# yixuan/ADMM

Hardware: AMD Instinct MI355X
Metric: ADMM iterations/sec, Lasso tall n=100000 p=10000 (100-lambda warm-started path) (higher is better)
Workload: dtype f32; 1 GPU; admm_lasso tall path (BASELINE configs[1]); n=100000, p=10000, nlambda=100, standardize=True, intercept=True, parallelism=single GPU, step=one cold-started warm-chained lambda path

## Files before the change

admm_amd/_lib.py:

```python
import ctypes
import os

import numpy as np

_HERE = os.path.dirname(os.path.abspath(__file__))
LIB_PATH = os.environ.get("ADMM_HIP_LIB") or os.path.join(_HERE, "lib", "libadmm_hip.so")

ADMM_MEM_HOST = 0
ADMM_MEM_DEVICE = 1


class AdmmOpts(ctypes.Structure):
    _fields_ = [("maxit", ctypes.c_int), ("eps_abs", ctypes.c_double),
                ("eps_rel", ctypes.c_double), ("rho", ctypes.c_double)]


class AdmmHipOptions(ctypes.Structure):
    _fields_ = [(k, ctypes.c_int) for k in (
        "struct_size", "gram_backend", "gram_split", "factor_backend", "inverse_precision", "tall_xupdate", "tall_refine",
        "consensus_two_pass", "consensus_unfused", "bp_two_pass", "lad_no_hat", "wide_no_persist", "wide_unfused", "wide_gram_sprad",
        "sharing_bp_direct", "cv_downdate", "peer_exchange", "batch_iters", "profile_stride", "pool_mb", "screen", "lad_two_pass",
        "par_devices")] + [("reserved", ctypes.c_int * 9)]


# ... 30 lines not shown
           "admm_hip_device_synchronize", "admm_hip_lasso_plan_create", "admm_hip_lasso_plan_run",
           "admm_hip_lasso_plan_destroy", "admm_hip_comm_unique_id", "admm_hip_comm_init", "admm_hip_comm_finalize", "admm_hip_comm_info",
           "admm_hip_parlasso_dist", "admm_hip_lasso_plan_create_dist",
           "admm_hip_lasso_plan_trace_enable", "admm_hip_lasso_plan_trace_read",
           "admm_hip_lasso_plan_state_enable", "admm_hip_lasso_plan_state_read", "admm_hip_lasso_plan_system_read",
           "admm_hip_host_lanczos", "admm_hip_test_symv",
           "admm_hip_comm_peer_prepare", "admm_hip_comm_init_peer", "admm_hip_comm_init_shm", "admm_hip_comm_test_allreduce", "admm_hip_comm_test_reduce_scatter",
           "admm_hip_lasso_dist", "admm_hip_test_gram", "admm_hip_test_spd_inverse", "admm_hip_test_cv_fold_system",
           "admm_hip_lasso_dist_cols", "admm_hip_test_gemv_t", "admm_hip_lad_traced", "admm_hip_bp_traced",
           "admm_hip_lasso_plan_create_dist_cols", "admm_hip_lasso_cv", "admm_hip_lasso_multi",
           "admm_hip_parbp", "admm_hip_parbp_traced", "admm_hip_parbp_dist", "admm_hip_dantzig", "admm_hip_dantzig_traced",
           "admm_hip_lad_state", "admm_hip_bp_state", "admm_hip_lasso_plan_data_read", "admm_hip_trim_memory", "admm_hip_test_gather",
           "admm_hip_options_default", "admm_hip_options_set", "admm_hip_option_set", "admm_hip_options_reset", "admm_hip_option_get",
           "admm_hip_last_parallel_layout", "admm_hip_parallel_assign", "admm_hip_grplasso", "admm_hip_grplasso_plan_create",
           "admm_hip_quantreg", "admm_hip_quantreg_state",
           "admm_hip_mtlasso", "admm_hip_mtlasso_plan_create", "admm_hip_test_symv_multi"]

GROUP_MAX = 1024
MT_MAX = 16
MT_RHS_BUILT = (2, 4, 8, 12)

TRACE_FIELDS = 12
TRACE_COLD, TRACE_CONVERGED, TRACE_ACCELERATE, TRACE_RESTART = -1, 0, 1, 2
TRACE_CONTINUE = 1


def load():
    global _lib
    if _lib is not None:
        return _lib
    path = os.environ.get("ADMM_HIP_LIB") or LIB_PATH
# ... 127 lines not shown
    lib.admm_hip_lasso_plan_trace_read.argtypes = [ctypes.c_void_p, _c_double_p, ctypes.c_longlong, ctypes.POINTER(ctypes.c_longlong)]
    lib.admm_hip_lasso_plan_trace_read.restype = ctypes.c_int
    lib.admm_hip_lasso_plan_state_enable.argtypes = [ctypes.c_void_p, ctypes.c_longlong]
    lib.admm_hip_lasso_plan_state_enable.restype = ctypes.c_int
    lib.admm_hip_lasso_plan_state_read.argtypes = [ctypes.c_void_p, ctypes.POINTER(ctypes.c_float), ctypes.c_longlong,
                                                   ctypes.POINTER(ctypes.c_longlong), ctypes.POINTER(ctypes.c_longlong)]
    lib.admm_hip_lasso_plan_state_read.restype = ctypes.c_int
    lib.admm_hip_lasso_plan_data_read.argtypes = [ctypes.c_void_p, ctypes.POINTER(ctypes.c_float), ctypes.c_longlong, ctypes.POINTER(ctypes.c_float)]
    lib.admm_hip_lasso_plan_data_read.restype = ctypes.c_int
    lib.admm_hip_lasso_plan_system_read.argtypes = [ctypes.c_void_p, ctypes.POINTER(ctypes.c_float), ctypes.c_longlong]
    lib.admm_hip_lasso_plan_system_read.restype = ctypes.c_int
    lib.admm_hip_test_symv.argtypes = [_c_float_p, ctypes.c_int, _c_float_p, _c_float_p, _c_float_p, _c_float_p]
    lib.admm_hip_test_symv.restype = ctypes.c_int
    lib.admm_hip_test_symv_multi.argtypes = [_c_float_p, ctypes.c_int, _c_float_p, ctypes.c_int, ctypes.c_int, _c_float_p]
    lib.admm_hip_test_symv_multi.restype = ctypes.c_int
    lib.admm_hip_test_gram.argtypes = [ctypes.c_void_p, ctypes.c_int, ctypes.c_int, ctypes.c_int, ctypes.c_int, ctypes.c_void_p]
    lib.admm_hip_test_gram.restype = ctypes.c_int
    lib.admm_hip_test_gemv_t.argtypes = [ctypes.c_void_p, ctypes.c_int, ctypes.c_int, ctypes.c_int, ctypes.c_void_p, ctypes.c_void_p]
    lib.admm_hip_test_gemv_t.restype = ctypes.c_int
    lib.admm_hip_test_spd_inverse.argtypes = [ctypes.c_void_p, ctypes.c_int, ctypes.c_int, ctypes.c_void_p]
    lib.admm_hip_test_spd_inverse.restype = ctypes.c_int
    lib.admm_hip_test_cv_fold_system.argtypes = [ctypes.c_void_p, ctypes.c_void_p, ctypes.c_int, ctypes.c_int, ctypes.c_void_p, ctypes.c_int, ctypes.c_int,
                                                 ctypes.c_int, ctypes.c_int, ctypes.c_void_p, ctypes.c_void_p, ctypes.c_void_p, ctypes.c_void_p, ctypes.c_void_p]
    lib.admm_hip_test_cv_fold_system.restype = ctypes.c_int
    lib.admm_hip_host_lanczos.argtypes = [_c_float_p, ctypes.c_int, _c_float_p, _c_int_p]
    lib.admm_hip_host_lanczos.restype = ctypes.c_int
    lib.admm_hip_test_gather.argtypes = [ctypes.c_void_p, ctypes.c_int, ctypes.c_int, ctypes.c_int, ctypes.c_void_p, _c_double_p]
    lib.admm_hip_test_gather.restype = ctypes.c_int
    lib.admm_hip_last_parallel_layout.argtypes = [_c_int_p, _c_int_p, ctypes.c_int]
    lib.admm_hip_last_parallel_layout.restype = ctypes.c_int
# ... 87 lines not shown
```

admm_amd/csrc/api.hip:

```cpp
#include "calls.h"
#include "comm.h"
#include "inproc.h"
#include "test_hooks.h"

using namespace admm;

template <typename F>
static int guarded(F&& f) {
    try {
        check_option_overlay();
        f();
        return ADMM_OK;
    } catch (const Error& e) {
        set_last_error(e.what());
        return e.code;
    } catch (const std::bad_alloc&) {
        set_last_error("host allocation failed");
        return ADMM_ERR_INTERNAL;
    } catch (const std::exception& e) {
        set_last_error(e.what());
        return ADMM_ERR_INTERNAL;
    }
}

// ... 468 lines not shown

int admm_hip_test_symv(const float* A, int p, const float* v0, const float* v1, float* y0, float* y1) {
    return guarded([&] {
        ADMM_REQUIRE(A && v0 && v1 && y0 && y1 && p > 0, "bad arguments");
        test_symv(A, p, v0, v1, y0, y1);
    });
}

int admm_hip_test_symv_multi(const float* A, int p, const float* V, int nr, int rhs_per_pass, float* Yout) {
    return guarded([&] {
        ADMM_REQUIRE(A && V && Yout && p > 0 && nr >= 1 && nr <= 64, "bad arguments");
        test_symv_multi(A, p, V, nr, rhs_per_pass, Yout);
    });
}

int admm_hip_test_gram(const void* A, int rows, int cols, int atA, int is_double, void* G) {
    return guarded([&] {
        ADMM_REQUIRE(A && G && rows > 0 && cols > 0, "bad arguments");
        if (is_double) test_gram<double>(static_cast<const double*>(A), rows, cols, atA != 0, static_cast<double*>(G));
        else test_gram<float>(static_cast<const float*>(A), rows, cols, atA != 0, static_cast<float*>(G));
    });
}

int admm_hip_test_gemv_t(const void* A, int rows, int cols, int is_double, const void* v, void* y) {
    return guarded([&] {
        ADMM_REQUIRE(A && v && y && rows > 0 && cols > 0, "bad arguments");
        if (is_double) test_gemv_t<double>(static_cast<const double*>(A), rows, cols, static_cast<const double*>(v), static_cast<double*>(y));
        else test_gemv_t<float>(static_cast<const float*>(A), rows, cols, static_cast<const float*>(v), static_cast<float*>(y));
    });
}
// ... 24 lines not shown
```

admm_amd/csrc/lasso_tall.hip:

```cpp
#include "prep.h"
#include "gemv_kernels.h"
#include "symv_kernels.h"
#include "solvers.h"
#include "comm.h"
#include "loop_driver.h"
#include "plan_host.h"
#include "peer_device.h"
#include "probe.h"

namespace admm {

struct TallCtl {
    double rho, lam, eps_primal, eps_dual, adj_a, adj_c, tau;
    double a_next, tau_next;
    int mode;
    int restart;
    int iter;
    int lam_idx;
    int done;
    int first;
    int total;
    int fin_idx;
    int fin_niter;
    int pad;
// ... 11 lines not shown
    float* x; float* z0; float* z1; float* y0; float* y1; float* adj_z; float* adj_y; float* u; float* w;
    TallCtl* ctl;
    double* P;
    float* beta;
    int* niter;
    int* done_host;
#ifdef ADMM_HIP_PROBE
    long long* probe;
#endif
    double* trace;
    long long trace_cap;
    const float* refine_ab;
    long long refine_ld;
    float* state;
    long long state_cap;
};

constexpr int kTailThreads = 256;
constexpr int kTailLanes = kSySumLanes;
constexpr int kTailElems = kTailThreads / kTailLanes;

__device__ __forceinline__ double tall_load_partial(const double* p, bool in_launch) {
    if (!in_launch) return *p;
    return __longlong_as_double((long long)__hip_atomic_load(reinterpret_cast<const unsigned long long*>(p), __ATOMIC_RELAXED, __HIP_MEMORY_SCOPE_AGENT));
}
__device__ __forceinline__ void tall_store_wt(float* p, float v) {
    __hip_atomic_store(reinterpret_cast<unsigned int*>(p), __float_as_uint(v), __ATOMIC_RELAXED, __HIP_MEMORY_SCOPE_AGENT);
}
__device__ __forceinline__ void tall_store_wt(double* p, double v) {
    __hip_atomic_store(reinterpret_cast<unsigned long long*>(p), (unsigned long long)__double_as_longlong(v), __ATOMIC_RELAXED, __HIP_MEMORY_SCOPE_AGENT);
}
// ... 46 lines not shown
            out.mode = 1;
            out.iter = in.iter + 1;
            if (in.iter + 1 >= q.maxit) {
                out.fin_idx = in.lam_idx; out.fin_niter = q.maxit + 1;
            }
        }
        if (out.fin_idx >= 0) {
            out.lam_idx = in.lam_idx + 1;
            out.iter = 0;
            if (out.lam_idx >= q.nlam) out.done = 1;
            else out.lam = q.lambdas[out.lam_idx];
            q.niter[out.fin_idx] = out.fin_niter;
        }
    } else {
        out.mode = 1; out.tau = 0.0; out.restart = 0;
    }
    out.eps_primal = fmax(sqrt(x2), sqrt(z2)) * q.eps_rel + q.sqrt_p * q.eps_abs;
    out.eps_dual = sqrt(y2) * q.eps_rel + q.sqrt_p * q.eps_abs;
    out.a_next = 0.5 + 0.5 * sqrt(1.0 + 4.0 * out.adj_a * out.adj_a);
    out.tau_next = (out.adj_a - 1.0) / out.a_next;
    out.total = in.total + 1;
    *outp = out;
    if (out.done) *q.done_host = 1;
    WIDE_PROBE(3);
    WIDE_PROBE_FLUSH(2, in.total);
    if (q.trace != nullptr && in.total < q.trace_cap) {
        double* t = q.trace + (size_t)in.total * ADMM_TRACE_FIELDS;
        t[0] = in.lam_idx; t[1] = in.iter; t[2] = in.eps_primal; t[3] = in.eps_dual; t[4] = tr_rp; t[5] = tr_rd;
        t[6] = tr_c; t[7] = in.adj_c; t[8] = tr_code; t[9] = in.rho; t[10] = in.rho; t[11] = in.lam;
    }
// ... 425 lines not shown

__global__ void tall_init_kernel(TallParams q, double rho, double lam0) {
    const int i = blockIdx.x * blockDim.x + threadIdx.x;
    if (i < q.p) {
        q.x[i] = 0.f; q.z0[i] = 0.f; q.z1[i] = 0.f; q.y0[i] = 0.f; q.y1[i] = 0.f;
        q.adj_z[i] = 0.f; q.adj_y[i] = 0.f; q.u[i] = q.XY[i]; q.w[i] = 0.f;
    }
    if (i < 2 * q.nwg * 8) q.P[i] = 0.0;
    if (i == 0) {
        TallCtl c;
        c.rho = rho; c.lam = lam0; c.eps_primal = 0.0; c.eps_dual = 0.0;
        c.adj_a = 1.0; c.adj_c = 9999.0; c.tau = 0.0;
        c.a_next = 0.5 + 0.5 * sqrt(5.0); c.tau_next = 0.0;
        c.mode = 1; c.restart = 0; c.iter = 0; c.lam_idx = 0; c.done = 0; c.first = 1; c.total = 0; c.fin_idx = -1; c.fin_niter = 0; c.pad = 0;
        q.ctl[0] = c; q.ctl[1] = c;
    }
}

struct TallPlan final : LassoPlan {
    DeviceData<float> d;
    LassoProblem pb;
    hipStream_t st;
    admm_stats setup_stats{};
    int p = 0, nlam = 0, nwg = 0;
    long long ldp = 0;
    double rho = 0;
    std::vector<double> lam_user, lam_int;
    GemvTPlan pl;
    SymvPlan sy;
    bool use_sym = false;
    bool shard = false;
    bool peer_fused = false;
    bool peer_one = false;
    int exchange_code = 0;
    CommInfo ci;
    DevBuf<float> ab;
    double dist_flops = 0;
    long long ldv = 0;
    DevBuf<float> XY, M, a_part, b_part, x, z0, z1, y0, y1, adj_z, adj_y, u, w, beta;
    DevBuf<int> niter;
    DevBuf<double> P, dlam;
    DevBuf<TallCtl> ctl;
    TallParams q{};
    bool refine = false;
    DevBuf<float> Mg, rab, ruw;
    DevBuf<double> dD0, dD1, xD0, xD1;
    bool grouped = false;
    DevBuf<int2> gtiles;
    DevBuf<GroupCoord> gcoord;
    GroupTailParams gq{};
    int mt = 0;
    int mt_rhs = 2;
    DevBuf<float> uw, mdot, maxp;
    DevBuf<double> roww;
    MtTailParams mq{};
    PinnedFlag hflag;
#ifdef ADMM_HIP_PROBE
// ... 186 lines not shown
        u.zero(st); w.zero(st);
        ADMM_HIP_CHECK(hipMemcpyAsync(dlam.get(), lam_int.data(), nlam * sizeof(double), hipMemcpyHostToDevice, st));

        q.p = p; q.nwg = nwg; q.nseg = pl.nseg; q.maxit = pb.opts.maxit; q.nlam = nlam; q.enet = pb.enet ? 1 : 0;
        q.part_stride = ldp;
        q.eps_abs = pb.opts.eps_abs; q.eps_rel = pb.opts.eps_rel; q.alpha = (double)(float)pb.alpha; q.sqrt_p = std::sqrt((double)p * (double)npl);
        q.lambdas = dlam.get(); q.XY = XY.get(); q.a_part = a_part.get(); q.b_part = b_part.get();
        if (shard) { q.a_part = ab.get(); q.b_part = ab.get() + ldp; q.nseg = 1; }
        q.dot0 = sy.dot0.get(); q.dot1 = sy.dot1.get(); q.axp0 = sy.axp0.get(); q.axp1 = sy.axp1.get();
        q.ldo = sy.ldo; q.nrb = sy.nrb; q.p32 = sy.p32; q.sched = sy.sched;
        q.refine_ab = refine ? rab.get() : nullptr; q.refine_ld = ldv;
        q.x = x.get(); q.z0 = z0.get(); q.z1 = z1.get(); q.y0 = y0.get(); q.y1 = y1.get();
        q.adj_z = adj_z.get(); q.adj_y = adj_y.get(); q.u = u.get(); q.w = w.get();
        q.ctl = ctl.get(); q.P = P.get(); q.beta = beta.get(); q.niter = niter.get();
        q.done_host = hflag.p;
#ifdef ADMM_HIP_PROBE
        probe.alloc((size_t)4096 * 4 * 8); probe.zero(st);
        q.probe = probe.get();
        sy.probe = probe.get();
#endif

        if (mt) {
            static const int kAutoRhs[kMtMax] = {2, 4, 8, 8, 12, 12, 8, 8, 4, 4, 12, 12, 4, 4, 8, 8};
            mt_rhs = kAutoRhs[mt - 1];
            if (const OptValue* v = opt(Opt::MT_RHS)) { if (v->i > 0) mt_rhs = kSyNR[v->i - 1]; }
            uw.alloc((size_t)2 * mt * ldv); uw.zero(st);
            const size_t ds = (size_t)sy.nrb * sy.ldo, as = (size_t)sy.nax_rows * sy.ldo;
            mdot.alloc((size_t)2 * mt * ds); maxp.alloc((size_t)2 * mt * as);
            mdot.zero(st); maxp.zero(st);
            x.zero(st); z0.zero(st); z1.zero(st); y0.zero(st); y1.zero(st); adj_z.zero(st); adj_y.zero(st);
// ... 63 lines not shown

    void read_system(float* out, long long ld) override {
        if (!refine) throw Error(ADMM_ERR_INVALID_ARG, "the system matrix is only kept with ADMM_HIP_REFINE=1");
        ADMM_REQUIRE(out != nullptr && ld >= p, "bad output for the system matrix");
        ADMM_HIP_CHECK(hipMemcpy2D(out, (size_t)ld * sizeof(float), Mg.get(), (size_t)ldp * sizeof(float), (size_t)p * sizeof(float), (size_t)p, hipMemcpyDeviceToHost));
    }

    void run(LassoResult& res) override {
        admm_stats S = setup_stats;
        S.xupdate_variant = shard ? 2 : (use_sym ? 1 : 0);
        S.exchange_variant = exchange_code;
        S.refine = refine ? 1 : 0;
        S.factor_flops = dist_flops;
        res.lambda = lam_user;
        beta.zero(st); niter.zero(st);
        const int init_n = std::max(p, 2 * nwg * 8);
        for (int k = 0; k < std::max(mt, 1); ++k) {
            TallParams qk = q;
            if (mt) {
                const size_t o = (size_t)k * ldv;
                qk.x += o; qk.z0 += o; qk.z1 += o; qk.y0 += o; qk.y1 += o; qk.adj_z += o; qk.adj_y += o;
                qk.XY += (size_t)k * ldp; qk.u = uw.get() + (size_t)(2 * k) * ldv; qk.w = uw.get() + (size_t)(2 * k + 1) * ldv;
            }
            hipLaunchKernelGGL(tall_init_kernel, dim3((init_n + 255) / 256), dim3(256), 0, st, qk, rho, lam_int[0]);
        }
        if (q.state != nullptr && mt)
            ADMM_HIP_CHECK(hipMemcpy2DAsync(q.state, (size_t)p * sizeof(float), XY.get(), (size_t)ldp * sizeof(float), (size_t)p * sizeof(float),
                                            (size_t)mt, hipMemcpyDeviceToDevice, st));
        else if (q.state != nullptr)
            ADMM_HIP_CHECK(hipMemcpyAsync(q.state, XY.get(), (size_t)p * sizeof(float), hipMemcpyDeviceToDevice, st));
// ... 7 lines not shown
        size_t nev = 0;
        const auto done_at = [&](long long g) -> const int* { return &ctl.get()[(int)(g & 1)].done; };
        const LoopTimes lt = run_until_done(st, done_at, batch, (long long)nlam * ((long long)pb.opts.maxit + 2) + 4, [&](long long g) {
            const int par = (int)(g & 1);
            const bool sample = stride > 0 && (g % stride) == stride / 2 && nev < 8192;
            hipEvent_t e0 = nullptr, e1 = nullptr;
            if (sample) {
                while (ev_pool.size() < nev + 2) {
                    hipEvent_t e; ADMM_HIP_CHECK(hipEventCreate(&e));
                    ev_pool.push_back(e);
                }
                e0 = ev_pool[nev]; e1 = ev_pool[nev + 1];
                nev += 2;
            }
            const TallDecideExtra dec{q, par};
            if (mt) {
                const int nvec = 2 * mt;
                for (int r0 = 0; r0 < nvec; r0 += mt_rhs) {
                    SymvNArgs a;
                    a.A = M.get(); a.lda = ldp; a.p = p;
                    a.v = uw.get() + (size_t)r0 * ldv; a.vstride = ldv;
                    a.dot = mdot.get() + (size_t)r0 * mq.dot_stride; a.dot_stride = mq.dot_stride;
                    a.axp = maxp.get() + (size_t)r0 * mq.axp_stride; a.axp_stride = mq.axp_stride;
                    a.nvec = std::min(mt_rhs, nvec - r0); a.ldo = sy.ldo; a.tiles = sy.tiles.get(); a.skip = &ctl.get()[par].done;
                    hipEvent_t es = r0 == 0 ? e0 : nullptr, ee = r0 + mt_rhs >= nvec ? e1 : nullptr;
                    if (r0 == 0) symvn_launch(sy, mt_rhs, a, st, dec, es, ee);
                    else symvn_launch(sy, mt_rhs, a, st, SymvNoExtra(), es, ee);
                }
                hipLaunchKernelGGL(tall_mt_tail_kernel, dim3(nwg), dim3(kTailThreads), 0, st, q, par, mq);
            } else if (grouped) {
                if (use_sym) {
                    sy.launch(M.get(), ldp, u.get(), w.get(), &ctl.get()[par].done, st, dec, e0, e1);
                    hipLaunchKernelGGL(tall_group_tail_kernel<TAIL_SYMV>, dim3(nwg), dim3(kTailThreads), 0, st, q, par, gq);
                } else {
                    launch_gemv_t<float, 2, 4, TallDecideExtra>(pl, M.get(), ldp, p, p, u.get(), w.get(), a_part.get(), b_part.get(), ldp,
                                                                &ctl.get()[par].done, st, dec, e0, e1);
                    hipLaunchKernelGGL(tall_group_tail_kernel<TAIL_GEMV>, dim3(nwg), dim3(kTailThreads), 0, st, q, par, gq);
                }
            } else if (shard && peer_fused) {
                sy.launch(M.get(), ldp, u.get(), w.get(), &ctl.get()[par].done, st, dec, e0, e1);
                const PeerExchange ex = comm_peer_begin((size_t)2 * ldp * sizeof(float));
                if (peer_one) {
                    hipLaunchKernelGGL(tall_tail_kernel<TAIL_PEER1>, dim3(nwg), dim3(kTailThreads), 0, st, q, par, ex);
                } else {
                    hipLaunchKernelGGL(tall_shard_push_kernel, dim3(nwg), dim3(kTailThreads), 0, st, q, ex, ldp, &ctl.get()[par].done);
                    hipLaunchKernelGGL(tall_tail_kernel<TAIL_PEER>, dim3(nwg), dim3(kTailThreads), 0, st, q, par, ex);
                }
// ... 3 lines not shown
                allreduce_sum_f32(ab.get(), (size_t)2 * ldp, st);
                hipLaunchKernelGGL(tall_tail_kernel<TAIL_GEMV>, dim3(nwg), dim3(kTailThreads), 0, st, q, par, PeerExchange{});
            } else if (use_sym && refine) {
                const int* skip = &ctl.get()[par].done;
                sy.launch(M.get(), ldp, u.get(), w.get(), skip, st, dec, e0, e1);
                hipLaunchKernelGGL(tall_shard_reduce_kernel, dim3(nwg), dim3(kTailThreads), 0, st, q, rab.get(), ldv, skip);
                SymvArgsD ad;
                ad.A = Mg.get(); ad.lda = ldp; ad.p = p; ad.v0 = rab.get(); ad.v1 = rab.get() + ldv;
                ad.dot0 = dD0.get(); ad.dot1 = dD1.get(); ad.axp0 = xD0.get(); ad.axp1 = xD1.get(); ad.ldo = sy.ldo; ad.tiles = sy.tiles.get(); ad.skip = skip;
                hipLaunchKernelGGL(symv2_lower_f64acc_kernel, dim3(sy.ntiles), dim3(kSyThreads), 0, st, ad);
                hipLaunchKernelGGL(tall_refine_resid_kernel, dim3(nwg), dim3(kTailThreads), 0, st, q, dD0.get(), dD1.get(), xD0.get(), xD1.get(),
                                   ruw.get(), ruw.get() + ldv, skip);
                sy.launch(M.get(), ldp, ruw.get(), ruw.get() + ldv, skip, st, SymvNoExtra());
                hipLaunchKernelGGL(tall_tail_kernel<TAIL_SYMV>, dim3(nwg), dim3(kTailThreads), 0, st, q, par, PeerExchange{});
            } else if (use_sym) {
                sy.launch(M.get(), ldp, u.get(), w.get(), &ctl.get()[par].done, st, dec, e0, e1);
                hipLaunchKernelGGL(tall_tail_kernel<TAIL_SYMV>, dim3(nwg), dim3(kTailThreads), 0, st, q, par, PeerExchange{});
            } else {
                launch_gemv_t<float, 2, 4, TallDecideExtra>(pl, M.get(), ldp, p, p, u.get(), w.get(), a_part.get(), b_part.get(), ldp,
                                                            &ctl.get()[par].done, st, dec, e0, e1);
                hipLaunchKernelGGL(tall_tail_kernel<TAIL_GEMV>, dim3(nwg), dim3(kTailThreads), 0, st, q, par, PeerExchange{});
            }
        }, LoopOpts{shard ? nullptr : hflag.p, 0, false});
        S.t_loop = lt.wall_s; S.loop_ms_events = lt.events_ms; S.xupdate_launches = lt.launched;
        const CtlPair<TallCtl> hctl = read_ctl(ctl.get());
        WIDE_PROBE_DUMP(probe);
        if (nev > 0) {
            double tot = 0;
            for (size_t k = 0; k + 1 < nev; k += 2) {
                float m1 = 0.f;
                ADMM_HIP_CHECK(hipEventElapsedTime(&m1, ev_pool[k], ev_pool[k + 1]));
                tot += m1;
            }
            S.xupdate_samples = (long long)(nev / 2);
            S.xupdate_ms_avg = tot / (double)(nev / 2);
        }

        ADMM_HIP_CHECK(hipMemcpyAsync(hbeta, beta.get(), (size_t)nlam * p * std::max(mt, 1) * sizeof(float), hipMemcpyDeviceToHost, st));
        comm_stream_sync(st);
        if (mt) {
// ... 21 lines not shown
```

admm_amd/csrc/options.h:

```cpp
#pragma once
#include <limits>
#include <string>
#include <vector>

namespace admm {

enum class OptKind { Flag, Int, Real, Choice, Text, Sched, Devices };
struct OptAccepts {
    OptKind kind;
    double lo = 0, hi = 0;
    const char* choices = nullptr;
};
constexpr OptAccepts Flag() { return {OptKind::Flag, 0, 1}; }
constexpr OptAccepts Int(double lo, double hi) { return {OptKind::Int, lo, hi}; }
constexpr OptAccepts Real(double lo, double hi) { return {OptKind::Real, lo, hi}; }
constexpr OptAccepts Choice(const char* c) { return {OptKind::Choice, 0, 0, c}; }
constexpr OptAccepts Text() { return {OptKind::Text}; }
constexpr OptAccepts Sched() { return {OptKind::Sched}; }
constexpr OptAccepts Devices() { return {OptKind::Devices}; }
constexpr double kPositive = std::numeric_limits<double>::min();

#define ADMM_OPTIONS(X)                                                                                                                  \
    X(BATCH_ITERS, Int(1, 1 << 20), "iterations enqueued between two host polls (rounded up to even; default per solver)")             \
    X(PROFILE_STRIDE, Int(0, 1 << 30), "time every k-th tall x-update launch with HIP events (0: off)")                                 \
    X(GRAM, Choice("rocblas|oneshot"), "tall Gram through rocBLAS / host input transferred before the Gram is built")                    \
    X(GRAM_SPLIT, Choice("0|f16x2|bf16x3"), "tall Gram of order >= ~4000: exact fp32 kernel / fp16 x 2 (default) / bf16 x 3")          \
    X(GRAM_B3_KTILES, Int(0, 1 << 20), "K tiles per launch of the 16-bit split Gram (0: one launch)")                                   \
    X(FACTOR, Choice("rocsolver"), "Cholesky + inverse through rocSOLVER / rocBLAS instead of the hand-written kernels")                \
    X(INVERSE, Choice("f32|f64"), "precision the cached inverse is built in")                                                           \
    X(XUPDATE, Choice("sym|gemv|full"), "tall x-update: symmetric lower-triangle kernel / full-matrix mat-vec (gemv and full alike)")   \
    X(SYMV_SCHED, Sched(), "tall x-update: column-segment widths of the long / short row strips and the split between them")           \
    X(REFINE, Flag(), "tall path: refine every x-update with a double-precision residual")                                               \
    X(DIST_FACTOR, Flag(), "row-sharded tall solver: 0 = every rank factorises the whole all-reduced Gram")                            \
    X(CV_DOWNDATE, Flag(), "cross-validation folds' Grams as down-dates of the full-data Gram: 1 always, 0 never")                      \
    X(PREP_FUSED, Flag(), "0: convert, column statistics and standardisation as separate sweeps over X")                                \
    X(H2D, Choice("pageable"), "host inputs through plain hipMemcpy instead of the pinned staging ring")                                 \
    X(POOL_MB, Int(0, 1 << 30), "cache of released device blocks, megabytes (0: off)")                                                  \
    X(WIDE_FUSE, Flag(), "wide path: 0 = three launches per iteration")                                                                  \
    X(WIDE_TGLOBAL, Flag(), "wide path: 1 = t through global memory instead of LDS")                                                     \
    X(WIDE_SPRAD, Choice("gram"), "wide path: spectral radius from the explicit n x n Gram")                                            \
    X(WIDE_SCREEN, Choice("0|8|16|auto"), "wide path: screen the regular steps never / 8-bit code / fp16 copy / chosen at any size")    \
    X(WIDE_SCREEN_STATS, Flag(), "wide path: print the screen's counts")                                                                 \
    X(WIDE_PERSIST, Flag(), "wide path: 0 = no persistent active-set stretches")                                                         \
    X(WIDE_PERSIST_COLS, Flag(), "column-sharded wide solver: 0 = no persistent active-set stretches")                                  \
    X(WIDE_ROWS_C, Int(1, 32), "wide path: column groups of the 2-D stretch (kept only when it fits with the problem's row groups)")    \
    X(WIDE_PERSIST_STATS, Flag(), "wide path: print the stretch statistics")                                                             \
// ... 71 lines not shown
```

admm_amd/csrc/symv_kernels.h:

```cpp
#pragma once
#include "admm_internal.h"
#include "device_utils.h"
#include <hip/hip_ext.h>

namespace admm {

constexpr int kSyRB = 256;
constexpr int kSyCB = 128;
constexpr int kSyCBMax = 256;
static_assert(kSyCBMax == 256, "SYMV_SCHED's widths are checked against 256 where the option is parsed (options.hip)");
constexpr int kSyThreads = 256;

struct SymvSched {
    int width_big = kSyCB, width_small = kSyCB;
    int rb_split = 0;
    __host__ __device__ int width(int rb) const { return rb >= rb_split ? width_big : width_small; }
    __host__ __device__ int nseg(int rb, int p32) const {
        const int cols = min((rb + 1) * kSyRB, p32), w = width(rb);
        return (cols + w - 1) / w;
    }
};
constexpr int kSySumLanes = 8;

struct SymvArgs {
    const float* A; long long lda; int p;
    const float* v0; const float* v1;
    float* dot0; float* dot1;
    float* axp0; float* axp1;
    long long ldo;
    const int4* tiles;
    const int* skip;
#ifdef ADMM_HIP_PROBE
    long long* probe; int probe_idx;
#endif
};

template <typename T>
__device__ __forceinline__ T butterfly8(const T (&v)[8], int lane) {
    T a4[4], a2[2];
    {
        const int b = (lane >> 5) & 1;
#pragma unroll
        for (int k = 0; k < 4; ++k) {
            const T keep = b ? v[k + 4] : v[k], send = b ? v[k] : v[k + 4];
            a4[k] = keep + __shfl_xor(send, 32, 64);
        }
    }
    {
        const int b = (lane >> 4) & 1;
// ... 16 lines not shown
    __device__ __forceinline__ float4 load4(const float* p) const { return *reinterpret_cast<const float4*>(p); }
    __device__ __forceinline__ float load1(const float* p) const { return *p; }
};
struct SymvBypassVec {
    __device__ __forceinline__ float4 load4(const float* p) const {
        const unsigned long long lo = __hip_atomic_load(reinterpret_cast<const unsigned long long*>(p), __ATOMIC_RELAXED, __HIP_MEMORY_SCOPE_AGENT);
        const unsigned long long hi = __hip_atomic_load(reinterpret_cast<const unsigned long long*>(p) + 1, __ATOMIC_RELAXED, __HIP_MEMORY_SCOPE_AGENT);
        return make_float4(__uint_as_float((unsigned)lo), __uint_as_float((unsigned)(lo >> 32)), __uint_as_float((unsigned)hi), __uint_as_float((unsigned)(hi >> 32)));
    }
    __device__ __forceinline__ float load1(const float* p) const {
        return __uint_as_float(__hip_atomic_load(reinterpret_cast<const unsigned int*>(p), __ATOMIC_RELAXED, __HIP_MEMORY_SCOPE_AGENT));
    }
};
struct SymvNoWait { __device__ __forceinline__ void operator()() const {} };

template <bool PRE, typename Wait, typename VecLoad, bool NT = false>
__device__ __forceinline__ void symv2_tile(const SymvArgs& a, const int4 t, Wait wait, VecLoad vl,
                                           float4 (*red)[kSyThreads], float (*sdot)[kSyCBMax]) {
    const int rb = t.x, seg = t.w;
    const int cw = t.z >> 2;
    const int lane = threadIdx.x & 63, wid = threadIdx.x >> 6;
    const int row = rb * kSyRB + lane * 4;
    const int col0 = t.y + wid * cw;
    const int p4 = (a.p + 3) & ~3;
    const bool active = row < p4;
    const bool has = col0 < a.p;
    const float* base = a.A + (size_t)col0 * a.lda + row;
    float4 av[8];
    if (PRE) {
#pragma unroll
        for (int k = 0; k < 8; ++k) {
            av[k] = make_float4(0.f, 0.f, 0.f, 0.f);
            if (has && active && col0 + k < a.p) av[k] = *reinterpret_cast<const float4*>(base + (size_t)k * a.lda);
        }
        wait();
    }
    float4 aU = make_float4(0.f, 0.f, 0.f, 0.f), aW = aU;

    if (has) {
        const float4 uI = active ? vl.load4(a.v0 + row) : make_float4(0.f, 0.f, 0.f, 0.f);
        const float4 wI = active ? vl.load4(a.v1 + row) : make_float4(0.f, 0.f, 0.f, 0.f);
        const int cj = col0 + lane;
        const float uj = (lane < cw && cj < a.p) ? vl.load1(a.v0 + cj) : 0.f;
        const float wj = (lane < cw && cj < a.p) ? vl.load1(a.v1 + cj) : 0.f;
        const bool diag = col0 + (cw - 1) >= rb * kSyRB;
        const int nq = cw >> 3;
#pragma unroll 1
        for (int q = 0; q < nq; ++q) {
            if (!PRE || q > 0) {
#pragma unroll
                for (int k = 0; k < 8; ++k) {
                    const int col = col0 + q * 8 + k;
                    av[k] = make_float4(0.f, 0.f, 0.f, 0.f);
                    if constexpr (NT) { if (active && col < a.p) av[k] = load16_nt<float4>(base + (size_t)(q * 8 + k) * a.lda); }
                    else { if (active && col < a.p) av[k] = *reinterpret_cast<const float4*>(base + (size_t)(q * 8 + k) * a.lda); }
                }
            }
            float dU[8], dW[8];
#pragma unroll
            for (int k = 0; k < 8; ++k) {
                const int col = col0 + q * 8 + k;
                float4 v = av[k];
                float4 ax = v;
                if (diag) {
                    if (row + 0 < col) v.x = 0.f;
                    if (row + 1 < col) v.y = 0.f;
                    if (row + 2 < col) v.z = 0.f;
                    if (row + 3 < col) v.w = 0.f;
                    ax = v;
                    if (row + 0 == col) ax.x = 0.f;
                    if (row + 1 == col) ax.y = 0.f;
// ... 25 lines not shown
#pragma unroll
        for (int ww = 1; ww < 4; ++ww) {
            const float4 o = red[wid][ww * 64 + lane];
            s.x += o.x; s.y += o.y; s.z += o.z; s.w += o.w;
        }
        float* dst = (wid == 0 ? a.axp0 : a.axp1) + (size_t)seg * a.ldo + row;
        *reinterpret_cast<float4*>(dst) = s;
    } else {
        float* dst = (wid == 2 ? a.dot0 : a.dot1) + (size_t)rb * a.ldo + t.y;
        for (int c = lane * 4; c < t.z; c += 256) *reinterpret_cast<float4*>(dst + c) = *reinterpret_cast<const float4*>(&sdot[wid - 2][c]);
    }
}

struct SymvNoExtra { __device__ void operator()() const {} };

template <typename Extra, bool NT = false>
__global__ void __launch_bounds__(kSyThreads, 4)
symv2_lower_kernel(SymvArgs a, Extra extra) {
    if (blockIdx.x == 0) { extra(); return; }
    if (a.skip != nullptr && *a.skip != 0) return;
    __shared__ float4 red[2][kSyThreads];
    __shared__ __attribute__((aligned(16))) float sdot[2][kSyCBMax];
#ifdef ADMM_HIP_PROBE
    const long long pt0 = wall_clock64();
#endif
    symv2_tile<false, SymvNoWait, SymvPlainVec, NT>(a, a.tiles[blockIdx.x - 1], SymvNoWait(), SymvPlainVec(), red, sdot);
#ifdef ADMM_HIP_PROBE
    if (a.probe != nullptr && threadIdx.x == 0) {
        const int nt = (int)gridDim.x - 1, t = (int)blockIdx.x - 1;
        const int which = t == 0 ? 0 : (t == nt / 2 ? 1 : (t == nt - 1 ? 2 : (t == (3 * nt) / 4 ? 3 : -1)));
        if (which >= 0) {
            long long* d = a.probe + ((size_t)(a.probe_idx & 4095) * 4 + 3) * 8 + which * 2;
            d[0] = pt0; d[1] = wall_clock64();
        }
    }
#endif
}

struct SymvNArgs {
    const float* A; long long lda; int p;
    const float* v; long long vstride;
// ... 196 lines not shown
    } else {
        double* dst = (wid == 2 ? a.dot0 : a.dot1) + (size_t)rb * a.ldo + t.y;
        for (int c = lane; c < t.z; c += 64) dst[c] = sdot[wid - 2][c];
    }
}

struct SymvPlan {
    int p = 0, nrb = 0, ncb = 0, ntiles = 0, p32 = 0;
    int nax_rows = 0;
    SymvSched sched;
    long long ldo = 0;
    DevBuf<int4> tiles;
    std::vector<int4> htiles;
    bool nt = false;
    DevBuf<float> dot0, dot1, axp0, axp1;
#ifdef ADMM_HIP_PROBE
    long long* probe = nullptr; mutable int probe_idx = 0;
#endif
    void init(int p_, hipStream_t st, int part = 0, int nparts = 1) {
        p = p_;
        p32 = (p + 31) / 32 * 32;
        nrb = (p + kSyRB - 1) / kSyRB;
        ncb = (p + kSyCB - 1) / kSyCB;
        ldo = (long long)nrb * kSyRB;
        auto count = [&](const SymvSched& sc) { long long t = 0; for (int rb = 0; rb < nrb; ++rb) t += sc.nseg(rb, p32); return t; };
        int cus = 256;
        { int dev = 0; hipDeviceProp_t prop; if (hipGetDevice(&dev) == hipSuccess && hipGetDeviceProperties(&prop, dev) == hipSuccess) cus = prop.multiProcessorCount; }
        const long long slots = 4ll * cus * std::max(1, nparts);
        auto uniform = [](int w) { SymvSched sc; sc.width_big = sc.width_small = w; sc.rb_split = 0; return sc; };
        auto two = [&](int wb, int ws) { SymvSched sc; sc.width_big = wb; sc.width_small = ws; sc.rb_split = nrb / 2; return sc; };
// ... 24 lines not shown
                const int gw = w / gcd(w, 128) * 128;
                const int cg = t.y / gw;
                if (t.x != last_rb || cg != last_cg) { ++group; last_rb = t.x; last_cg = cg; }
                if (group % nparts == part) mine.push_back(t);
            }
            h.swap(mine);
        }
        ntiles = (int)h.size();
        htiles = h;
        nt = (size_t)2 * (size_t)p * (size_t)p / (size_t)std::max(1, nparts) > (size_t)310000000;
        tiles.alloc(std::max<size_t>(h.size(), 1));
        if (!h.empty()) ADMM_HIP_CHECK(hipMemcpyAsync(tiles.get(), h.data(), h.size() * sizeof(int4), hipMemcpyHostToDevice, st));
        dot0.alloc((size_t)nrb * ldo); dot1.alloc((size_t)nrb * ldo);
        axp0.alloc((size_t)nax_rows * ldo); axp1.alloc((size_t)nax_rows * ldo);
        dot0.zero(st); dot1.zero(st); axp0.zero(st); axp1.zero(st);
        ADMM_HIP_CHECK(hipStreamSynchronize(st));
    }
    SymvArgs args(const float* A, long long lda, const float* v0, const float* v1, const int* skip) const {
        SymvArgs a;
        a.A = A; a.lda = lda; a.p = p; a.v0 = v0; a.v1 = v1;
        a.dot0 = dot0.get(); a.dot1 = dot1.get(); a.axp0 = axp0.get(); a.axp1 = axp1.get();
        a.ldo = ldo; a.tiles = tiles.get(); a.skip = skip;
#ifdef ADMM_HIP_PROBE
        a.probe = probe; a.probe_idx = probe_idx++;
#endif
        return a;
    }
    template <typename Extra = SymvNoExtra>
    void launch(const float* A, long long lda, const float* v0, const float* v1, const int* skip, hipStream_t st, Extra extra = Extra(),
                hipEvent_t ev_start = nullptr, hipEvent_t ev_stop = nullptr) {
        const SymvArgs a = args(A, lda, v0, v1, skip);
        if (nt) {
            if (ev_start == nullptr && ev_stop == nullptr) hipLaunchKernelGGL((symv2_lower_kernel<Extra, true>), dim3(ntiles + 1), dim3(kSyThreads), 0, st, a, extra);
            else hipExtLaunchKernelGGL((symv2_lower_kernel<Extra, true>), dim3(ntiles + 1), dim3(kSyThreads), 0, st, ev_start, ev_stop, 0, a, extra);
            return;
        }
        if (ev_start == nullptr && ev_stop == nullptr) hipLaunchKernelGGL((symv2_lower_kernel<Extra>), dim3(ntiles + 1), dim3(kSyThreads), 0, st, a, extra);
        else hipExtLaunchKernelGGL((symv2_lower_kernel<Extra>), dim3(ntiles + 1), dim3(kSyThreads), 0, st, ev_start, ev_stop, 0, a, extra);
    }
};

template <int NL, typename T = float>
__device__ __forceinline__ void symv_sum_partials(const T* __restrict__ dot0, const T* __restrict__ dot1,
                                                  const T* __restrict__ axp0, const T* __restrict__ axp1,
                                                  long long ldo, int nrb, const SymvSched sched, int p32, int i, int sub, bool valid, T& a, T& b) {
    const int ic = valid ? i : 0;
    const int rbi = ic / kSyRB;
    const int rb0 = rbi;
    const int ndot = nrb - rb0;
// ... 93 lines not shown
```

include/admm_hip.h:

```cpp
#ifndef ADMM_HIP_H
#define ADMM_HIP_H

#ifdef __cplusplus
extern "C" {
#endif

#if defined(__GNUC__)
#define ADMM_HIP_API __attribute__((visibility("default")))
#else
#define ADMM_HIP_API
#endif

#define ADMM_OK 0
#define ADMM_ERR_INVALID_ARG 1
#define ADMM_ERR_NO_DEVICE 2
#define ADMM_ERR_HIP 3
#define ADMM_ERR_BLAS 4
#define ADMM_ERR_NOT_SPD 5
#define ADMM_ERR_EIGS 6
#define ADMM_ERR_COMM 7
#define ADMM_ERR_INTERNAL 8
#define ADMM_ERR_MEMORY 9

#define ADMM_MEM_HOST 0
// ... 215 lines not shown
ADMM_HIP_API int admm_hip_parallel_assign(int nblocks, const char* par_devices, int device_count, int* nranks, int* devices, int cap);

ADMM_HIP_API const char* admm_hip_last_error(void);
ADMM_HIP_API const char* admm_hip_version(void);
ADMM_HIP_API int admm_hip_trim_memory(void);
ADMM_HIP_API int admm_hip_device_count(void);
ADMM_HIP_API int admm_hip_set_device(int device);
ADMM_HIP_API int admm_hip_device_synchronize(void);



ADMM_HIP_API int admm_hip_host_lanczos(const float* A, int n, float* eig_out, int* nmatop_out);

ADMM_HIP_API int admm_hip_test_symv(const float* A, int p, const float* v0, const float* v1, float* y0, float* y1);
ADMM_HIP_API int admm_hip_test_symv_multi(const float* A, int p, const float* V, int nr, int rhs_per_pass, float* Yout);

ADMM_HIP_API int admm_hip_test_gram(const void* A, int rows, int cols, int atA, int is_double, void* G);
ADMM_HIP_API int admm_hip_test_gemv_t(const void* A, int rows, int cols, int is_double, const void* v, void* y);
ADMM_HIP_API int admm_hip_test_gather(const void* A, int rows, int cols, int is_double, const void* v, double* y);
ADMM_HIP_API int admm_hip_test_spd_inverse(const void* A, int n, int precision, void* Ainv);
ADMM_HIP_API int admm_hip_test_cv_fold_system(const double* x, const double* y, int n, int p, const int* fold_id, int nfolds, int fold,
                                              int standardize, int intercept, float* gram, float* xy, float* mean_x, float* scale_x,
                                              float* mean_scale_y);

#ifdef __cplusplus
}
#endif
#endif
```

Baseline: 25520 iterations/s.

## Let symv tiles exit early when the decide block discards the launch

Block 0 of the symmetric x-update kernel decides whether the iteration converged or restarts. When it does, it now writes a run-tagged verdict word to 64 replicated slots. Other tiles check this word at start, and by default also between column chunks, and exit early, which saves the HBM reads of the large Gram inverse for speculatively launched work that will be thrown away. The change also narrows each load to the actual last valid column on diagonal tiles. It adds an atomic load per chunk and a counter of early exits; a wrong tag or a race could drop work that was still needed.

After: 26180 iterations/s (median of 6 runs). 2.6% higher.

```diff
diff --git a/admm_amd/_lib.py b/admm_amd/_lib.py
--- a/admm_amd/_lib.py
+++ b/admm_amd/_lib.py
@@ -68,7 +68,7 @@
            "admm_hip_options_default", "admm_hip_options_set", "admm_hip_option_set", "admm_hip_options_reset", "admm_hip_option_get",
            "admm_hip_last_parallel_layout", "admm_hip_parallel_assign", "admm_hip_grplasso", "admm_hip_grplasso_plan_create",
            "admm_hip_quantreg", "admm_hip_quantreg_state",
-           "admm_hip_mtlasso", "admm_hip_mtlasso_plan_create", "admm_hip_test_symv_multi"]
+           "admm_hip_mtlasso", "admm_hip_mtlasso_plan_create", "admm_hip_test_symv_multi", "admm_hip_test_tall_early_exits"]
 
 GROUP_MAX = 1024
 MT_MAX = 16
@@ -226,6 +226,8 @@
     lib.admm_hip_test_symv.restype = ctypes.c_int
     lib.admm_hip_test_symv_multi.argtypes = [_c_float_p, ctypes.c_int, _c_float_p, ctypes.c_int, ctypes.c_int, _c_float_p]
     lib.admm_hip_test_symv_multi.restype = ctypes.c_int
+    lib.admm_hip_test_tall_early_exits.argtypes = [ctypes.POINTER(ctypes.c_longlong)]
+    lib.admm_hip_test_tall_early_exits.restype = ctypes.c_int
     lib.admm_hip_test_gram.argtypes = [ctypes.c_void_p, ctypes.c_int, ctypes.c_int, ctypes.c_int, ctypes.c_int, ctypes.c_void_p]
     lib.admm_hip_test_gram.restype = ctypes.c_int
     lib.admm_hip_test_gemv_t.argtypes = [ctypes.c_void_p, ctypes.c_int, ctypes.c_int, ctypes.c_int, ctypes.c_void_p, ctypes.c_void_p]
diff --git a/admm_amd/csrc/api.hip b/admm_amd/csrc/api.hip
--- a/admm_amd/csrc/api.hip
+++ b/admm_amd/csrc/api.hip
@@ -506,6 +506,13 @@
     });
 }
 
+int admm_hip_test_tall_early_exits(long long* count) {
+    return guarded([&] {
+        ADMM_REQUIRE(count != nullptr, "bad arguments");
+        *count = tall_last_early_exits();
+    });
+}
+
 int admm_hip_test_gram(const void* A, int rows, int cols, int atA, int is_double, void* G) {
     return guarded([&] {
         ADMM_REQUIRE(A && G && rows > 0 && cols > 0, "bad arguments");
diff --git a/admm_amd/csrc/lasso_tall.hip b/admm_amd/csrc/lasso_tall.hip
--- a/admm_amd/csrc/lasso_tall.hip
+++ b/admm_amd/csrc/lasso_tall.hip
@@ -49,7 +49,15 @@
     long long refine_ld;
     float* state;
     long long state_cap;
+    unsigned long long* verdict;
+    unsigned long long run_tag;
 };
+
+__host__ __device__ inline unsigned long long tall_verdict_word(unsigned long long run_tag, int total, bool discard) {
+    return run_tag | ((unsigned long long)(unsigned)total << 1) | (discard ? 1ull : 0ull);
+}
+constexpr int kVerdictShift = 33;
+constexpr int kVerdictWords = kSyVerdictReplicas * kSyVerdictStride;
 
 constexpr int kTailThreads = 256;
 constexpr int kTailLanes = kSySumLanes;
@@ -126,6 +134,11 @@
         }
     } else {
         out.mode = 1; out.tau = 0.0; out.restart = 0;
+    }
+    if (q.verdict != nullptr && (out.mode == 0 || out.done)) {
+        const unsigned long long word = tall_verdict_word(q.run_tag, in.total + 1, true);
+        for (int r = 0; r < kSyVerdictReplicas; ++r)
+            __hip_atomic_store(q.verdict + (size_t)r * kSyVerdictStride, word, __ATOMIC_RELAXED, __HIP_MEMORY_SCOPE_AGENT);
     }
     out.eps_primal = fmax(sqrt(x2), sqrt(z2)) * q.eps_rel + q.sqrt_p * q.eps_abs;
     out.eps_dual = sqrt(y2) * q.eps_rel + q.sqrt_p * q.eps_abs;
@@ -581,8 +594,12 @@
         c.a_next = 0.5 + 0.5 * sqrt(5.0); c.tau_next = 0.0;
         c.mode = 1; c.restart = 0; c.iter = 0; c.lam_idx = 0; c.done = 0; c.first = 1; c.total = 0; c.fin_idx = -1; c.fin_niter = 0; c.pad = 0;
         q.ctl[0] = c; q.ctl[1] = c;
-    }
-}
+        if (q.verdict != nullptr) q.verdict[kVerdictWords] = 0;
+    }
+}
+
+static thread_local long long t_early_exits = 0;
+long long tall_last_early_exits() { return t_early_exits; }
 
 struct TallPlan final : LassoPlan {
     DeviceData<float> d;
@@ -608,6 +625,9 @@
     DevBuf<int> niter;
     DevBuf<double> P, dlam;
     DevBuf<TallCtl> ctl;
+    DevBuf<unsigned long long> verdict;
+    bool verdict_on = false, verdict_mid = false;
+    unsigned long long run_no = 0;
     TallParams q{};
     bool refine = false;
     DevBuf<float> Mg, rab, ruw;
@@ -824,6 +844,12 @@
         q.adj_z = adj_z.get(); q.adj_y = adj_y.get(); q.u = u.get(); q.w = w.get();
         q.ctl = ctl.get(); q.P = P.get(); q.beta = beta.get(); q.niter = niter.get();
         q.done_host = hflag.p;
+        verdict_on = use_sym && !shard && !refine && !mt && !opt_off(Opt::SYMV_VERDICT);
+        verdict_mid = opt_int(Opt::SYMV_VERDICT, 2) == 2;
+        if (verdict_on) {
+            verdict.alloc(kVerdictWords + kSyVerdictStride); verdict.zero(st);
+            q.verdict = verdict.get();
+        }
 #ifdef ADMM_HIP_PROBE
         probe.alloc((size_t)4096 * 4 * 8); probe.zero(st);
         q.probe = probe.get();
@@ -917,6 +943,7 @@
         S.factor_flops = dist_flops;
         res.lambda = lam_user;
         beta.zero(st); niter.zero(st);
+        q.run_tag = ++run_no << kVerdictShift;
         const int init_n = std::max(p, 2 * nwg * 8);
         for (int k = 0; k < std::max(mt, 1); ++k) {
             TallParams qk = q;
@@ -954,6 +981,8 @@
                 nev += 2;
             }
             const TallDecideExtra dec{q, par};
+            SymvVerdict vd;
+            if (verdict_on) { vd.words = verdict.get(); vd.discard = tall_verdict_word(q.run_tag, (int)(g + 1), true); vd.early = verdict.get() + kVerdictWords; vd.mid = verdict_mid; }
             if (mt) {
                 const int nvec = 2 * mt;
                 for (int r0 = 0; r0 < nvec; r0 += mt_rhs) {
@@ -970,7 +999,7 @@
                 hipLaunchKernelGGL(tall_mt_tail_kernel, dim3(nwg), dim3(kTailThreads), 0, st, q, par, mq);
             } else if (grouped) {
                 if (use_sym) {
-                    sy.launch(M.get(), ldp, u.get(), w.get(), &ctl.get()[par].done, st, dec, e0, e1);
+                    sy.launch(M.get(), ldp, u.get(), w.get(), &ctl.get()[par].done, st, dec, e0, e1, vd);
                     hipLaunchKernelGGL(tall_group_tail_kernel<TAIL_SYMV>, dim3(nwg), dim3(kTailThreads), 0, st, q, par, gq);
                 } else {
                     launch_gemv_t<float, 2, 4, TallDecideExtra>(pl, M.get(), ldp, p, p, u.get(), w.get(), a_part.get(), b_part.get(), ldp,
@@ -1004,7 +1033,7 @@
                 sy.launch(M.get(), ldp, ruw.get(), ruw.get() + ldv, skip, st, SymvNoExtra());
                 hipLaunchKernelGGL(tall_tail_kernel<TAIL_SYMV>, dim3(nwg), dim3(kTailThreads), 0, st, q, par, PeerExchange{});
             } else if (use_sym) {
-                sy.launch(M.get(), ldp, u.get(), w.get(), &ctl.get()[par].done, st, dec, e0, e1);
+                sy.launch(M.get(), ldp, u.get(), w.get(), &ctl.get()[par].done, st, dec, e0, e1, vd);
                 hipLaunchKernelGGL(tall_tail_kernel<TAIL_SYMV>, dim3(nwg), dim3(kTailThreads), 0, st, q, par, PeerExchange{});
             } else {
                 launch_gemv_t<float, 2, 4, TallDecideExtra>(pl, M.get(), ldp, p, p, u.get(), w.get(), a_part.get(), b_part.get(), ldp,
@@ -1014,6 +1043,9 @@
         }, LoopOpts{shard ? nullptr : hflag.p, 0, false});
         S.t_loop = lt.wall_s; S.loop_ms_events = lt.events_ms; S.xupdate_launches = lt.launched;
         const CtlPair<TallCtl> hctl = read_ctl(ctl.get());
+        unsigned long long early = 0;
+        if (verdict_on) ADMM_HIP_CHECK(hipMemcpy(&early, verdict.get() + kVerdictWords, sizeof early, hipMemcpyDeviceToHost));
+        t_early_exits = (long long)early;
         WIDE_PROBE_DUMP(probe);
         if (nev > 0) {
             double tot = 0;
diff --git a/admm_amd/csrc/options.h b/admm_amd/csrc/options.h
--- a/admm_amd/csrc/options.h
+++ b/admm_amd/csrc/options.h
@@ -30,6 +30,7 @@
     X(INVERSE, Choice("f32|f64"), "precision the cached inverse is built in")                                                           \
     X(XUPDATE, Choice("sym|gemv|full"), "tall x-update: symmetric lower-triangle kernel / full-matrix mat-vec (gemv and full alike)")   \
     X(SYMV_SCHED, Sched(), "tall x-update: column-segment widths of the long / short row strips and the split between them")           \
+    X(SYMV_VERDICT, Choice("0|1|2"), "tall x-update: tiles of a discarded launch leave never / when they start / also mid-tile (default)") \
     X(REFINE, Flag(), "tall path: refine every x-update with a double-precision residual")                                               \
     X(DIST_FACTOR, Flag(), "row-sharded tall solver: 0 = every rank factorises the whole all-reduced Gram")                            \
     X(CV_DOWNDATE, Flag(), "cross-validation folds' Grams as down-dates of the full-data Gram: 1 always, 0 never")                      \
diff --git a/admm_amd/csrc/symv_kernels.h b/admm_amd/csrc/symv_kernels.h
--- a/admm_amd/csrc/symv_kernels.h
+++ b/admm_amd/csrc/symv_kernels.h
@@ -2,6 +2,7 @@
 #include "admm_internal.h"
 #include "device_utils.h"
 #include <hip/hip_ext.h>
+#include <climits>
 
 namespace admm {
 
@@ -30,9 +31,21 @@
     long long ldo;
     const int4* tiles;
     const int* skip;
+    const unsigned long long* verdict;
+    unsigned long long discard;
+    unsigned long long* early;
 #ifdef ADMM_HIP_PROBE
     long long* probe; int probe_idx;
 #endif
+};
+
+constexpr int kSyVerdictReplicas = 64;
+constexpr int kSyVerdictStride = 16;
+struct SymvVerdict {
+    const unsigned long long* words = nullptr;
+    unsigned long long discard = 0;
+    unsigned long long* early = nullptr;
+    bool mid = false;
 };
 
 template <typename T>
@@ -79,7 +92,7 @@
 };
 struct SymvNoWait { __device__ __forceinline__ void operator()() const {} };
 
-template <bool PRE, typename Wait, typename VecLoad, bool NT = false>
+template <bool PRE, typename Wait, typename VecLoad, bool NT = false, bool MID = false>
 __device__ __forceinline__ void symv2_tile(const SymvArgs& a, const int4 t, Wait wait, VecLoad vl,
                                            float4 (*red)[kSyThreads], float (*sdot)[kSyCBMax]) {
     const int rb = t.x, seg = t.w;
@@ -110,16 +123,24 @@
         const float wj = (lane < cw && cj < a.p) ? vl.load1(a.v1 + cj) : 0.f;
         const bool diag = col0 + (cw - 1) >= rb * kSyRB;
         const int nq = cw >> 3;
+        const int last = active ? min(a.p - 1, diag ? row + 3 : INT_MAX) : -1;
+        const unsigned long long* vword = a.verdict + (size_t)(blockIdx.x & (kSyVerdictReplicas - 1)) * kSyVerdictStride;
 #pragma unroll 1
         for (int q = 0; q < nq; ++q) {
+            unsigned long long vq = 0;
+            if constexpr (MID) vq = __hip_atomic_load(vword, __ATOMIC_RELAXED, __HIP_MEMORY_SCOPE_AGENT);
             if (!PRE || q > 0) {
 #pragma unroll
                 for (int k = 0; k < 8; ++k) {
                     const int col = col0 + q * 8 + k;
                     av[k] = make_float4(0.f, 0.f, 0.f, 0.f);
-                    if constexpr (NT) { if (active && col < a.p) av[k] = load16_nt<float4>(base + (size_t)(q * 8 + k) * a.lda); }
-                    else { if (active && col < a.p) av[k] = *reinterpret_cast<const float4*>(base + (size_t)(q * 8 + k) * a.lda); }
+                    if constexpr (NT) { if (col <= last) av[k] = load16_nt<float4>(base + (size_t)(q * 8 + k) * a.lda); }
+                    else { if (col <= last) av[k] = *reinterpret_cast<const float4*>(base + (size_t)(q * 8 + k) * a.lda); }
                 }
+            }
+            if constexpr (MID) {
+                const unsigned lo = __builtin_amdgcn_readfirstlane((unsigned)vq), hi = __builtin_amdgcn_readfirstlane((unsigned)(vq >> 32));
+                if ((((unsigned long long)hi << 32) | lo) == a.discard) break;
             }
             float dU[8], dW[8];
 #pragma unroll
@@ -175,17 +196,25 @@
 
 struct SymvNoExtra { __device__ void operator()() const {} };
 
-template <typename Extra, bool NT = false>
+template <typename Extra, bool NT = false, bool MID = false>
 __global__ void __launch_bounds__(kSyThreads, 4)
 symv2_lower_kernel(SymvArgs a, Extra extra) {
     if (blockIdx.x == 0) { extra(); return; }
-    if (a.skip != nullptr && *a.skip != 0) return;
+    const int4 t = a.tiles[blockIdx.x - 1];
+    const unsigned long long vw = __hip_atomic_load(a.verdict + (size_t)(blockIdx.x & (kSyVerdictReplicas - 1)) * kSyVerdictStride,
+                                                    __ATOMIC_RELAXED, __HIP_MEMORY_SCOPE_AGENT);
+    const int done = *a.skip;
+    if (done != 0) return;
+    if (vw == a.discard) {
+        if (threadIdx.x == 0) atomicAdd(a.early, 1ull);
+        return;
+    }
     __shared__ float4 red[2][kSyThreads];
     __shared__ __attribute__((aligned(16))) float sdot[2][kSyCBMax];
 #ifdef ADMM_HIP_PROBE
     const long long pt0 = wall_clock64();
 #endif
-    symv2_tile<false, SymvNoWait, SymvPlainVec, NT>(a, a.tiles[blockIdx.x - 1], SymvNoWait(), SymvPlainVec(), red, sdot);
+    symv2_tile<false, SymvNoWait, SymvPlainVec, NT, MID>(a, t, SymvNoWait(), SymvPlainVec(), red, sdot);
 #ifdef ADMM_HIP_PROBE
     if (a.probe != nullptr && threadIdx.x == 0) {
         const int nt = (int)gridDim.x - 1, t = (int)blockIdx.x - 1;
@@ -412,6 +441,7 @@
     std::vector<int4> htiles;
     bool nt = false;
     DevBuf<float> dot0, dot1, axp0, axp1;
+    DevBuf<unsigned long long> zero;
 #ifdef ADMM_HIP_PROBE
     long long* probe = nullptr; mutable int probe_idx = 0;
 #endif
@@ -466,13 +496,18 @@
         dot0.alloc((size_t)nrb * ldo); dot1.alloc((size_t)nrb * ldo);
         axp0.alloc((size_t)nax_rows * ldo); axp1.alloc((size_t)nax_rows * ldo);
         dot0.zero(st); dot1.zero(st); axp0.zero(st); axp1.zero(st);
+        zero.alloc((size_t)kSyVerdictReplicas * kSyVerdictStride); zero.zero(st);
         ADMM_HIP_CHECK(hipStreamSynchronize(st));
     }
-    SymvArgs args(const float* A, long long lda, const float* v0, const float* v1, const int* skip) const {
+    SymvArgs args(const float* A, long long lda, const float* v0, const float* v1, const int* skip, const SymvVerdict& vd = SymvVerdict()) const {
         SymvArgs a;
         a.A = A; a.lda = lda; a.p = p; a.v0 = v0; a.v1 = v1;
         a.dot0 = dot0.get(); a.dot1 = dot1.get(); a.axp0 = axp0.get(); a.axp1 = axp1.get();
-        a.ldo = ldo; a.tiles = tiles.get(); a.skip = skip;
+        a.ldo = ldo; a.tiles = tiles.get();
+        a.skip = skip != nullptr ? skip : reinterpret_cast<const int*>(zero.get());
+        a.verdict = vd.words != nullptr ? vd.words : zero.get();
+        a.discard = vd.words != nullptr ? vd.discard : ~0ull;
+        a.early = vd.early;
 #ifdef ADMM_HIP_PROBE
         a.probe = probe; a.probe_idx = probe_idx++;
 #endif
@@ -480,11 +515,16 @@
     }
     template <typename Extra = SymvNoExtra>
     void launch(const float* A, long long lda, const float* v0, const float* v1, const int* skip, hipStream_t st, Extra extra = Extra(),
-                hipEvent_t ev_start = nullptr, hipEvent_t ev_stop = nullptr) {
-        const SymvArgs a = args(A, lda, v0, v1, skip);
+                hipEvent_t ev_start = nullptr, hipEvent_t ev_stop = nullptr, const SymvVerdict& vd = SymvVerdict()) {
+        const SymvArgs a = args(A, lda, v0, v1, skip, vd);
         if (nt) {
             if (ev_start == nullptr && ev_stop == nullptr) hipLaunchKernelGGL((symv2_lower_kernel<Extra, true>), dim3(ntiles + 1), dim3(kSyThreads), 0, st, a, extra);
             else hipExtLaunchKernelGGL((symv2_lower_kernel<Extra, true>), dim3(ntiles + 1), dim3(kSyThreads), 0, st, ev_start, ev_stop, 0, a, extra);
+            return;
+        }
+        if (vd.words != nullptr && vd.mid) {
+            if (ev_start == nullptr && ev_stop == nullptr) hipLaunchKernelGGL((symv2_lower_kernel<Extra, false, true>), dim3(ntiles + 1), dim3(kSyThreads), 0, st, a, extra);
+            else hipExtLaunchKernelGGL((symv2_lower_kernel<Extra, false, true>), dim3(ntiles + 1), dim3(kSyThreads), 0, st, ev_start, ev_stop, 0, a, extra);
             return;
         }
         if (ev_start == nullptr && ev_stop == nullptr) hipLaunchKernelGGL((symv2_lower_kernel<Extra>), dim3(ntiles + 1), dim3(kSyThreads), 0, st, a, extra);
diff --git a/include/admm_hip.h b/include/admm_hip.h
--- a/include/admm_hip.h
+++ b/include/admm_hip.h
@@ -253,6 +253,7 @@
 
 ADMM_HIP_API int admm_hip_test_symv(const float* A, int p, const float* v0, const float* v1, float* y0, float* y1);
 ADMM_HIP_API int admm_hip_test_symv_multi(const float* A, int p, const float* V, int nr, int rhs_per_pass, float* Yout);
+ADMM_HIP_API int admm_hip_test_tall_early_exits(long long* count);
 
 ADMM_HIP_API int admm_hip_test_gram(const void* A, int rows, int cols, int atA, int is_double, void* G);
 ADMM_HIP_API int admm_hip_test_gemv_t(const void* A, int rows, int cols, int is_double, const void* v, void* y);
```
